# Geunwoo-Jeon/LarvaNet

Hardware: AMD Instinct MI355X
Metric: HR Mpixels/s (LarvaNet x4 multi-exit train step, 48x48 LR patches) (higher is better)
Workload: dtype f32; 1 GPU; LarvaNet x4 train_step_larva M4 B4,4,4,4 48ch, batch 16 of 3x48x48 -> 3x192x192 fp32 per GPU (BASELINE config 2); global_batch=16, parallelism=dp1, hip_graph=True

## Files before the change

larvanet_amd/csrc/conv3x3_mfma.hip:

```cpp
#include "larva_common.h"
#include "larva_bicubic.h"
#include <hip/hip_ext.h>
#include <cstdlib>
#include <type_traits>

#ifndef LARVA_DIAG
#define LARVA_DIAG 0
#endif
constexpr int kWgPerCu = 2;
constexpr int kOperandDepth = 2;


#ifndef LARVA_DIAG_ONLY48
#define LARVA_DIAG_ONLY48 0
#endif

namespace larva {

#if defined(LARVA_DIAG) && (LARVA_DIAG & 32)
__device__ unsigned long long* g_stamps = nullptr;
#if LARVA_DIAG & 512
constexpr int kDiagWgPerSlot = 256;
__device__ int g_slot_of_launch = 0;
__device__ __forceinline__ void stamp_slot(unsigned long long* area, int k) {
// ... 236 lines not shown

template <int COUT, typename G>
__device__ __forceinline__ void reg_load(const ConvArgs& a, const ChunkSrc& cs, int y0, int x0, int tid,
                                         RegStaging<COUT, G>& st) {
  using C = ConvCfg<COUT, G>;
  const size_t plane = (size_t)a.H * a.pitch;
#pragma unroll
  for (int i = 0; i < C::RIN_ITERS; ++i) {
    const int s = min(tid + i * 256, C::RIN_SLOTS - 1);
    const int ci = s / (G::HALO * (G::RS / 4));
    const int rem = s - ci * (G::HALO * (G::RS / 4));
    const int r = rem / (G::RS / 4);
    const int q = rem - r * (G::RS / 4);
    const int gy = y0 - 1 + r, gx = x0 - 4 + 4 * q;
    const bool row_ok = gy >= 0 && gy < a.H;
    const float* row = cs.img_ptr + (size_t)ci * plane + (size_t)min(max(gy, 0), a.H - 1) * a.pitch;
    f32x4 v;
#pragma unroll
    for (int e = 0; e < 4; ++e) {
      const int x = gx + e;
      const float t = row[min(max(x, 0), a.W - 1)];
      v[e] = (row_ok && x >= 0 && x < a.W) ? t : 0.f;
    }
    st.in[i] = v;
  }
#pragma unroll
  for (int i = 0; i < C::RW_ITERS; ++i) {
    const int s = min(tid + i * 256, C::RW_SLOTS - 1);
    const float* p = cs.wgt_ptr + 4 * s;
    st.w[i] = f32x4{p[0], p[1], p[2], p[3]};
  }
}

template <int COUT, typename G>
__device__ __forceinline__ void reg_store(float* stage, int tid, const RegStaging<COUT, G>& st) {
  using C = ConvCfg<COUT, G>;
#pragma unroll
  for (int i = 0; i < C::RIN_ITERS; ++i) {
    const int s = tid + i * 256;
    if (s < C::RIN_SLOTS) {
      const int ci = s / (G::HALO * (G::RS / 4));
      const int rem = s - ci * (G::HALO * (G::RS / 4));
      const int r = rem / (G::RS / 4);
      const int q = rem - r * (G::RS / 4);
      *reinterpret_cast<f32x4*>(stage + ci * C::PS + r * G::RS + 4 * q) = st.in[i];
    }
  }
#pragma unroll
  for (int i = 0; i < C::RW_ITERS; ++i) {
    const int s = tid + i * 256;
    if (s < C::RW_SLOTS) *reinterpret_cast<f32x4*>(stage + C::IN_FLOATS + 4 * s) = st.w[i];
  }
}

template <int COUT, typename G, int NCT, int PG0, int NPG>
__device__ __forceinline__ void read_operands(const float* const (&a_base)[NCT], const float* b_base, int step,
                                              float (&av)[NCT], float (&bv)[NPG]) {
  using C = ConvCfg<COUT, G>;
  if constexpr ((LARVA_DIAG & 128) != 0) {
#pragma unroll
    for (int c = 0; c < NCT; ++c) av[c] = (float)step;
#pragma unroll
    for (int p = 0; p < NPG; ++p) bv[p] = (float)(step + p);
    return;
  }
  const int tap = step / (kCh / 4), kk = step % (kCh / 4);
  const int ky = tap / 3, kx = tap % 3;
#pragma unroll
  for (int c = 0; c < NCT; ++c) av[c] = a_base[c][(tap * kCh + kk * 4) * C::CS];
#pragma unroll
  for (int p = 0; p < NPG; ++p) {
    const int pg = PG0 + p, prow = pg / G::PC, pcol = pg % G::PC;
    bv[p] = b_base[kk * 4 * C::PS + (prow + ky) * G::RS + pcol * 16 + kx];
  }
}

template <int NMF, int NRD, int M>
__device__ __forceinline__ void shadow_groups() {
  if constexpr (M < NMF) {
    __builtin_amdgcn_sched_group_barrier(0x8, 1, 0);
    constexpr int share = (NRD + NMF - 1 - M) / NMF;
    if constexpr (share > 0) __builtin_amdgcn_sched_group_barrier(0x100, share, 0);
    shadow_groups<NMF, NRD, M + 1>();
  }
}

template <int COUT, typename G, int NCT, int PG0, int NPG, bool SWAP>
__device__ __forceinline__ void mfma_chunk(const float* stage, int ct0, int lane, f32x4 (&acc)[NCT][NPG],
                                           const float* wstage = nullptr) {
  using C = ConvCfg<COUT, G>;
  const int lr = lane & 15, lq = lane >> 4;
  const float* const wrows = wstage ? wstage : stage + C::IN_FLOATS;
  const float* a_base[NCT];
#pragma unroll
  for (int c = 0; c < NCT; ++c)
    a_base[c] = wrows + lq * C::CS + lr + (cout_swizzled(COUT) ? (((ct0 + c) ^ (lq & 1)) * 16) : (ct0 + c) * 16);
  const float* b_base = stage + lq * C::PS + lr + 3;
  constexpr int D = kOperandDepth;
  float av[D + 1][NCT], bv[D + 1][NPG];
#pragma unroll
  for (int d = 0; d < D; ++d)
    if (d < C::STEPS) read_operands<COUT, G, NCT, PG0, NPG>(a_base, b_base, d, av[d], bv[d]);
#pragma unroll
  for (int step = 0; step < C::STEPS; ++step) {
    __builtin_amdgcn_sched_barrier(0);
    if (step + D < C::STEPS)
      read_operands<COUT, G, NCT, PG0, NPG>(a_base, b_base, step + D, av[(step + D) % (D + 1)], bv[(step + D) % (D + 1)]);
    constexpr int NMF = NCT * NPG;
    constexpr int NRD = NCT + NPG;
#pragma unroll
    for (int m = 0; m < NMF; ++m) {
      const float wv = av[step % (D + 1)][m / NPG], xv = bv[step % (D + 1)][m % NPG];
      acc[m / NPG][m % NPG] = __builtin_amdgcn_mfma_f32_16x16x4f32(SWAP ? xv : wv, SWAP ? wv : xv, acc[m / NPG][m % NPG], 0, 0, 0);
    }
    shadow_groups<NMF, NRD, 0>();
    __builtin_amdgcn_sched_barrier(0);
  }
}

template <int KEEP, int PIECES, int AUX>
__device__ __forceinline__ void wait_and_barrier() {
  static_assert(KEEP == PIECES + AUX, "a ring wait keeps exactly the next chunk's pieces and the operand loads in flight");
  asm volatile("; LARVA_RING pieces=%1 aux=%2\n\ts_waitcnt vmcnt(%0)\n\ts_barrier" ::"n"(KEEP), "n"(PIECES), "n"(AUX) : "memory");
  __builtin_amdgcn_sched_barrier(0);
}

template <typename G>
__device__ __forceinline__ void decode_tile(const ConvArgs& a, int vb, int& n, int& y0, int& x0) {
  const int tile = xcd_remap(vb, a.nwg);
  const int t2 = div_by_magic(tile, a.magic_tx);
  const int tx = tile - t2 * a.tiles_x;
  n = div_by_magic(t2, a.magic_ty);
  const int ty = t2 - n * a.tiles_y;
  x0 = tx * G::COLS;
  y0 = ty * G::ROWS;
}

template <int COUT, typename G, bool VEC, int EPI, int NCT, int PG0, int NPG, bool PERSIST>
struct RoleTraits {
  using C = ConvCfg<COUT, G>;
  static_assert(!VEC || C::LOADER, "the 16-byte path runs with a loader wave (2 * PIECES <= 63 for every instantiated shape)");
  static_assert(!PERSIST || VEC, "persistent tiles: the loader-wave path");
  static constexpr bool kShuffleEpi = (EPI == kEpiShuffle || EPI == kEpiShuffleBase || EPI == kEpiShuffleL1);
  static constexpr bool kPixMajor = VEC && !kShuffleEpi;
  static constexpr int NAUX = (EPI == kEpiMask || EPI == kEpiRes1 || EPI == kEpiShuffleBase)
                                  ? 1 : ((EPI == kEpiRes2 || EPI == kEpiShuffleL1) ? 2 : 0);
  static constexpr int NU = NCT * NPG;
  static constexpr int kEarlyPairs = PERSIST && COUT == 48 ? (NAUX * NU < 7 ? NAUX * NU : 7) : NAUX * NU;
  static constexpr int kLatePart = 4, kEarlyAll = 5;
  static constexpr bool kAuxLate = VEC && !kShuffleEpi && !(LARVA_DIAG & 6) && NAUX > 0 && !PERSIST;
  static constexpr int kAuxLoads = kAuxLate ? NAUX * NCT * NPG : 0;
};

template <int EPI, typename Aux>
__device__ __forceinline__ float fuse_element(float o, const Aux& aux, int c, int p, int r) {
  if constexpr (EPI == kEpiRelu) o = o < 0.f ? 0.f : o;
  if constexpr (EPI == kEpiMask) o = (aux[0][c][p][r] <= 0.f) ? 0.f : o;
  if constexpr (EPI == kEpiRes1 || EPI == kEpiRes2) o += aux[0][c][p][r];
  if constexpr (EPI == kEpiRes2) o += aux[1][c][p][r];
  return o;
}

template <int COUT, typename G, bool VEC, int EPI, int NCT, int PG0, int NPG, bool PERSIST = false>
__device__ __forceinline__ void run_role(const ConvArgs& a, float* smem, int ct0, int wave, int n, int y0, int x0, int tid) {
  using C = ConvCfg<COUT, G>;
  using T = RoleTraits<COUT, G, VEC, EPI, NCT, PG0, NPG, PERSIST>;
  constexpr bool kShuffleEpi = T::kShuffleEpi, kPixMajor = T::kPixMajor;
  constexpr int NAUX = T::NAUX;
  const int lane = tid & 63;
  const int lr = lane & 15, lq = lane >> 4;
  float* const out_ptr = a.out;
  struct { int H, W, pitch, plain; } k = {a.H, a.W, a.pitch, a.plain_stores};
  asm volatile("" : "+s"(k.H), "+s"(k.W), "+s"(k.pitch), "+s"(k.plain));

  f32x4 bias[NCT];
#pragma unroll
  for (int c = 0; c < NCT; ++c) bias[c] = f32x4{0.f, 0.f, 0.f, 0.f};
  auto load_bias = [&]() {
    if (a.bias) {
#pragma unroll
      for (int c = 0; c < NCT; ++c)
#pragma unroll
        for (int r = 0; r < 4; ++r) bias[c][r] = a.bias[(ct0 + c) * 16 + (kPixMajor ? lr : lq * 4 + r)];
    }
  };

  f32x4 aux[NAUX > 0 ? NAUX : 1][NAUX > 0 ? NCT : 1][NAUX > 0 ? NPG : 1];
  auto load_aux = [&](int part = -1) {
#pragma unroll
    for (int c = 0; c < NCT; ++c)
#pragma unroll
      for (int p = 0; p < NPG; ++p) {
        const int pg = PG0 + p, prow = pg / G::PC, pcol = pg % G::PC;
        const int y = min(y0 + prow, a.H - 1), x = min(x0 + pcol * 16 + lr, a.W - 1);
        auto want = [&](int op) {
          const int q = op * T::NU + c * NPG + p;
          return part < 0 ? true : part == T::kLatePart ? q >= T::kEarlyPairs : q < T::kEarlyPairs;
        };
        if constexpr (kShuffleEpi) {
          const int HH = 4 * a.H, WW = 4 * a.W;
          const size_t idx = (((size_t)n * C::CT + (ct0 + c)) * HH + (4 * y + lq)) * WW + 4 * x;
          if (want(0)) aux[0][c][p] = *reinterpret_cast<const f32x4*>(a.base + idx);
          if constexpr (EPI == kEpiShuffleL1) {
            if (want(1)) aux[1][c][p] = *reinterpret_cast<const f32x4*>(a.truth + idx);
          }
        } else if constexpr (kPixMajor && (PERSIST || G::COLS == 16)) {
          const unsigned plane = (unsigned)a.H * (unsigned)a.pitch;
          const unsigned lane_off = 4u * ((unsigned)lr * plane + (unsigned)lq * 4u);
          const int soff = __builtin_amdgcn_readfirstlane(
              (int)(4u * ((unsigned)((ct0 + c) * 16) * plane + (unsigned)(y0 + prow) * (unsigned)a.pitch + (unsigned)(x0 + pcol * 16))));
          auto image = [&](const float* t) {
            const unsigned long long b = reinterpret_cast<unsigned long long>(t + (size_t)n * COUT * plane);
            const unsigned lo = (unsigned)__builtin_amdgcn_readfirstlane((int)(unsigned)b);
            const unsigned hi = (unsigned)__builtin_amdgcn_readfirstlane((int)(unsigned)(b >> 32));
            return __builtin_amdgcn_make_buffer_rsrc(reinterpret_cast<void*>(((unsigned long long)hi << 32) | lo), 0,
                                                     (int)(COUT * plane * 4u), 0x00020000);
          };
          if constexpr (EPI == kEpiMask) {
            if (want(0)) aux[0][c][p] = __builtin_bit_cast(f32x4, __builtin_amdgcn_raw_buffer_load_b128(image(a.mask), lane_off, soff, 0));
          }
          if constexpr (EPI == kEpiRes1 || EPI == kEpiRes2) {
            if (want(0)) aux[0][c][p] = __builtin_bit_cast(f32x4, __builtin_amdgcn_raw_buffer_load_b128(image(a.res0), lane_off, soff, 0));
          }
          if constexpr (EPI == kEpiRes2) {
            if (want(1)) aux[1][c][p] = __builtin_bit_cast(f32x4, __builtin_amdgcn_raw_buffer_load_b128(image(a.res1), lane_off, soff, 0));
          }
        } else if constexpr (kPixMajor) {
          const size_t plane = (size_t)a.H * a.pitch;
          const int xb = min(x0 + pcol * 16 + lq * 4, a.pitch - 4);
          const size_t idx = ((size_t)n * COUT + (ct0 + c) * 16 + lr) * plane + (size_t)y * a.pitch + xb;
          if constexpr (EPI == kEpiMask) {
            if (want(0)) aux[0][c][p] = *reinterpret_cast<const f32x4*>(a.mask + idx);
          }
          if constexpr (EPI == kEpiRes1 || EPI == kEpiRes2) {
            if (want(0)) aux[0][c][p] = *reinterpret_cast<const f32x4*>(a.res0 + idx);
          }
          if constexpr (EPI == kEpiRes2) {
            if (want(1)) aux[1][c][p] = *reinterpret_cast<const f32x4*>(a.res1 + idx);
          }
        } else {
          const size_t plane = (size_t)a.H * a.pitch;
          const size_t idx0 = ((size_t)n * COUT + (ct0 + c) * 16 + lq * 4) * plane + (size_t)y * a.pitch + x;
#pragma unroll
          for (int r = 0; r < 4; ++r) {
            if constexpr (EPI == kEpiMask) aux[0][c][p][r] = a.mask[idx0 + r * plane];
            if constexpr (EPI == kEpiRes1 || EPI == kEpiRes2) aux[0][c][p][r] = a.res0[idx0 + r * plane];
            if constexpr (EPI == kEpiRes2) aux[1][c][p][r] = a.res1[idx0 + r * plane];
          }
        }
      }
  };
  auto load_early = [&]() {
    load_bias();
    if constexpr (NAUX > 0 && !T::kAuxLate && !(LARVA_DIAG & 4)) load_aux();
  };
  int pstage = 0;
  for (int vb = blockIdx.x;; vb += gridDim.x) {
  if constexpr (PERSIST) {
    if (vb >= a.nwg) break;
    decode_tile<G>(a, vb, n, y0, x0);
  }
  if constexpr (!VEC || (LARVA_DIAG & 2)) load_early();

  f32x4 acc[NCT][NPG];
#pragma unroll
  for (int c = 0; c < NCT; ++c)
#pragma unroll
    for (int p = 0; p < NPG; ++p) acc[c][p] = f32x4{0.f, 0.f, 0.f, 0.f};

  if constexpr (PERSIST) {
    load_bias();
    const int my_chunk = a.n_chunks >= 4 ? (wave & 3) : 0;
    __builtin_amdgcn_sched_barrier(0);
    for (int chunk = 0; chunk < a.n_chunks; ++chunk) {
      asm volatile("s_barrier" ::: "memory");
      __builtin_amdgcn_sched_barrier(0);
      if constexpr (NAUX > 0) {
        if (chunk == my_chunk) load_aux(T::kEarlyAll);
        __builtin_amdgcn_sched_barrier(0);
      }
      mfma_chunk<COUT, G, NCT, PG0, NPG, kPixMajor>(smem + pstage * C::STAGE_FLOATS, ct0, lane, acc);
      pstage = pstage == C::NST - 1 ? 0 : pstage + 1;
    }
    asm volatile("s_waitcnt vmcnt(0)" ::: "memory");
    __builtin_amdgcn_sched_barrier(0);
    if constexpr (T::kEarlyPairs < NAUX * T::NU) {
      load_aux(T::kLatePart);
      __builtin_amdgcn_sched_barrier(0);
    }
  } else if constexpr (VEC) {
    DmaPlan<COUT, G> pl;
    const int last = a.n_chunks - 1;
    if constexpr (!(LARVA_DIAG & 2)) {
      const ChunkSrc cs0 = chunk_src<COUT, G>(a, 0, n);
      const unsigned st0 = lds_addr_of(smem), st1 = lds_addr_of(smem + C::STAGE_FLOATS);
      stamp(6);
      make_plan<COUT, G, true>(a, wave, lane, y0, x0, pl);
#pragma unroll
      for (int i = 0; i < C::NPW; ++i)
        if (wave + 4 * i >= C::IN_PIECES) dma_piece<COUT, G>(pl, i, wave, cs0, st0);
      __builtin_amdgcn_sched_barrier(0);
      stamp(7);
      load_early();
      stamp(14);
      make_plan<COUT, G, false>(a, wave, lane, y0, x0, pl);
#pragma unroll
      for (int i = 0; i < C::NPW; ++i)
        if (wave + 4 * i < C::IN_PIECES) dma_piece<COUT, G>(pl, i, wave, cs0, st0);
      stamp(15);
      const ChunkSrc cs1 = chunk_src<COUT, G>(a, min(1, last), n);
#pragma unroll
      for (int i = 0; i < C::NPW; ++i) dma_piece<COUT, G>(pl, i, wave, cs1, st1);
      if constexpr (T::kAuxLate) {
        __builtin_amdgcn_sched_barrier(0);
        load_aux();
        __builtin_amdgcn_sched_barrier(0);
      }
    }
    stamp(1);
    int stage = 0;
    for (int chunk = 0; chunk <= last; ++chunk) {
      if constexpr ((LARVA_DIAG & 256) != 0) {
      } else if (chunk == 0) wait_and_barrier<((LARVA_DIAG & 2) ? 0 : C::NPW) + T::kAuxLoads, ((LARVA_DIAG & 2) ? 0 : C::NPW), T::kAuxLoads>();
      else wait_and_barrier<T::kAuxLoads, 0, T::kAuxLoads>();
      if (chunk == 0) stamp(2);
      stamp(8 + (chunk < 7 ? chunk : 7));
      if constexpr (!(LARVA_DIAG & 1)) mfma_chunk<COUT, G, NCT, PG0, NPG, kPixMajor>(smem + stage * C::STAGE_FLOATS, ct0, lane, acc);
      stage = stage == C::NST - 1 ? 0 : stage + 1;
    }
    asm volatile("s_waitcnt vmcnt(0)" ::: "memory");
    stamp(3);
  } else {
    RegStaging<COUT, G> st;
    if constexpr (!(LARVA_DIAG & 2)) {
      reg_load<COUT, G>(a, chunk_src<COUT, G>(a, 0, n), y0, x0, tid, st);
      reg_store<COUT, G>(smem, tid, st);
    }
    __syncthreads();
    for (int chunk = 0; chunk < a.n_chunks; ++chunk) {
      float* cur = smem + (chunk & 1) * C::STAGE_FLOATS;
      float* nxt = smem + ((chunk & 1) ^ 1) * C::STAGE_FLOATS;
      const bool more = chunk + 1 < a.n_chunks;
      if constexpr (!(LARVA_DIAG & 2)) {
        if (more) reg_load<COUT, G>(a, chunk_src<COUT, G>(a, chunk + 1, n), y0, x0, tid, st);
      }
      if constexpr (!(LARVA_DIAG & 1)) mfma_chunk<COUT, G, NCT, PG0, NPG, kPixMajor>(cur, ct0, lane, acc);
      if constexpr (!(LARVA_DIAG & 2)) {
        if (more) reg_store<COUT, G>(nxt, tid, st);
      }
      __syncthreads();
    }
  }

  if constexpr ((LARVA_DIAG & 4) != 0) {
#pragma unroll
    for (int c = 0; c < NCT; ++c)
#pragma unroll
      for (int p = 0; p < NPG; ++p) asm volatile("" ::"v"(acc[c][p]));
    return;
  }

  if constexpr (EPI == kEpiShuffleL1) {
    const int HH = 4 * k.H, WW = 4 * k.W;
    const size_t plane = (size_t)k.H * k.pitch;
    const float g = a.gval;
    float s = 0.f;
#pragma unroll
    for (int c = 0; c < NCT; ++c)
#pragma unroll
      for (int p = 0; p < NPG; ++p) {
        const int pg = PG0 + p, prow = pg / G::PC, pcol = pg % G::PC;
        const int y = y0 + prow, x = x0 + pcol * 16 + lr;
        const f32x4 v = (acc[c][p] + bias[c]) + aux[0][c][p];
        if (y < k.H && x < k.W) {
          if (out_ptr) {
            const size_t idx = (((size_t)n * C::CT + (ct0 + c)) * HH + (4 * y + lq)) * WW + 4 * x;
            __builtin_nontemporal_store(v, reinterpret_cast<f32x4*>(out_ptr + idx));
          }
          const f32x4 d = v - aux[1][c][p];
          s += fabsf(d[0]) + fabsf(d[1]) + fabsf(d[2]) + fabsf(d[3]);
          const size_t idx0 = ((size_t)n * COUT + (ct0 + c) * 16 + lq * 4) * plane + (size_t)y * k.pitch + x;
#pragma unroll
          for (int r = 0; r < 4; ++r)
            __builtin_nontemporal_store(d[r] > 0.f ? g : (d[r] < 0.f ? -g : 0.f), &a.grad[idx0 + r * plane]);
        }
      }
#pragma unroll
    for (int o = 32; o > 0; o >>= 1) s += __shfl_xor(s, o);
    if (lane == 0) a.partial[4 * blockIdx.x + wave] = s;
  } else if constexpr (EPI == kEpiShuffle || EPI == kEpiShuffleBase) {
    const int HH = 4 * k.H, WW = 4 * k.W;
#pragma unroll
    for (int c = 0; c < NCT; ++c)
#pragma unroll
      for (int p = 0; p < NPG; ++p) {
        const int pg = PG0 + p, prow = pg / G::PC, pcol = pg % G::PC;
        const int y = y0 + prow, x = x0 + pcol * 16 + lr;
        const size_t idx = (((size_t)n * C::CT + (ct0 + c)) * HH + (4 * y + lq)) * WW + 4 * x;
        f32x4 v = acc[c][p] + bias[c];
        if constexpr (EPI == kEpiShuffleBase) v += aux[0][c][p];
        if (y < k.H && x < k.W) __builtin_nontemporal_store(v, reinterpret_cast<f32x4*>(out_ptr + idx));
      }
  } else if constexpr (kPixMajor) {
    const size_t plane = (size_t)k.H * k.pitch;
    auto store_all = [&](auto plain_tag, auto interior_tag) {
      constexpr bool kPlain = decltype(plain_tag)::value;
      constexpr bool kInterior = decltype(interior_tag)::value;
#pragma unroll
      for (int c = 0; c < NCT; ++c)
#pragma unroll
        for (int p = 0; p < NPG; ++p) {
          const int pg = PG0 + p, prow = pg / G::PC, pcol = pg % G::PC;
          const int y = y0 + prow, xb = x0 + pcol * 16 + lq * 4;
          const size_t idx = ((size_t)n * COUT + (ct0 + c) * 16 + lr) * plane + (size_t)y * k.pitch + xb;
          f32x4 v = acc[c][p] + bias[c];
          if (kInterior || (y < k.H && xb < k.pitch)) {
#pragma unroll
            for (int r = 0; r < 4; ++r) {
              const float o = fuse_element<EPI>(v[r], aux, c, p, r);
              v[r] = (kInterior || xb + r < k.W) ? o : 0.f;
            }
            if constexpr (kPlain) *reinterpret_cast<f32x4*>(out_ptr + idx) = v;
            else __builtin_nontemporal_store(v, reinterpret_cast<f32x4*>(out_ptr + idx));
          }
        }
    };
    constexpr bool kFastPath = EPI == kEpiPlain || EPI == kEpiRelu || EPI == kEpiRes1;
    const bool interior = kFastPath && y0 + G::ROWS <= k.H && x0 + G::COLS <= k.W;
    auto store_policy = [&](auto plain_tag) {
      if constexpr (kFastPath) {
        if (interior) {
          store_all(plain_tag, std::true_type{});
          return;
        }
      }
      store_all(plain_tag, std::false_type{});
    };
    if constexpr ((LARVA_DIAG & 16) != 0) {
      store_policy(std::true_type{});
    } else if constexpr (G::COLS == 16) {
      if (k.plain) store_policy(std::true_type{});
      else store_policy(std::false_type{});
    } else {
      store_policy(std::false_type{});
    }
  } else {
    const size_t plane = (size_t)k.H * k.pitch;
#pragma unroll
    for (int c = 0; c < NCT; ++c)
#pragma unroll
      for (int p = 0; p < NPG; ++p) {
        const int pg = PG0 + p, prow = pg / G::PC, pcol = pg % G::PC;
        const int y = y0 + prow, x = x0 + pcol * 16 + lr;
        const size_t idx0 = ((size_t)n * COUT + (ct0 + c) * 16 + lq * 4) * plane + (size_t)y * k.pitch + x;
        const f32x4 v = acc[c][p] + bias[c];
        if (y < k.H && x < k.pitch) {
          const bool real = x < k.W;
#pragma unroll
          for (int r = 0; r < 4; ++r) {
            float o = fuse_element<EPI>(v[r], aux, c, p, r);
            o = real ? o : 0.f;
            if constexpr ((LARVA_DIAG & 16) != 0) out_ptr[idx0 + r * plane] = o;
            else __builtin_nontemporal_store(o, &out_ptr[idx0 + r * plane]);
          }
        }
      }
  }
#if LARVA_DIAG & 32
  stamp(4);
  asm volatile("s_waitcnt vmcnt(0)" ::: "memory");
  stamp(5);
#endif
  if constexpr (!PERSIST) break;
  }
}

__device__ __forceinline__ void fetch_args(const ConvArgs& a) {
  asm volatile("" ::"s"(a.src[0]), "s"(a.wpk), "s"(a.bias), "s"(a.out), "s"(a.cin_per_src), "s"(a.n_chunks), "s"(a.N),
               "s"(a.H), "s"(a.W), "s"(a.pitch), "s"(a.tiles_x), "s"(a.tiles_y), "s"(a.magic_tx), "s"(a.magic_ty),
               "s"(a.magic_cps), "s"(a.nwg), "s"(a.tile_tab), "s"(a.plain_stores), "s"(a.tab_n),
               "s"(a.tab16[0]), "s"(a.tab16[16]));
}

template <int COUT, bool VEC, int EPI, typename G = GeoWide, bool GIVEN = false>
__device__ __forceinline__ void conv_tile(const ConvArgs& a, float* smem, int wave = 0, int n = 0, int y0 = 0, int x0 = 0, int tid = 0) {
  static_assert(COUT == 48 || COUT == 32 || COUT == 64, "unsupported channel count");
  if constexpr (!GIVEN) {
    if constexpr ((LARVA_DIAG & 8) != 0) return;
    stamp(0);
    fetch_args(a);
    const int tile = xcd_remap(blockIdx.x, a.nwg);
    const int t2 = div_by_magic(tile, a.magic_tx);
    const int tx = tile - t2 * a.tiles_x;
    n = div_by_magic(t2, a.magic_ty);
    const int ty = t2 - n * a.tiles_y;
    x0 = tx * G::COLS, y0 = ty * G::ROWS;
    tid = threadIdx.x;
    wave = __builtin_amdgcn_readfirstlane(tid >> 6);
    __builtin_amdgcn_s_setprio(1);
  }
  if constexpr (VEC) {
    if (wave == 4) {
      if constexpr (GIVEN || !(LARVA_DIAG & 2)) run_loader<COUT, G>(a, smem, tid & 63, n, y0, x0);
      return;
    }
  }
  if constexpr (G::COLS == 16) {
    static_assert(VEC && ConvCfg<COUT, G>::LOADER, "the strip kernel is launched with a loader wave");
    if constexpr (COUT == 64) {
      run_role<COUT, G, VEC, EPI, 1, 0, G::ROWS>(a, smem, wave, wave, n, y0, x0, tid);
    } else if constexpr (COUT == 48) {
      if (wave < 3) run_role<COUT, G, VEC, EPI, 1, 0, G::ROWS - 1>(a, smem, wave, wave, n, y0, x0, tid);
      else run_role<COUT, G, VEC, EPI, 3, G::ROWS - 1, 1>(a, smem, 0, wave, n, y0, x0, tid);
    } else if constexpr (G::ROWS == 5) {
      if (wave < 2) run_role<COUT, G, VEC, EPI, 1, 0, 3>(a, smem, wave, wave, n, y0, x0, tid);
      else if (wave == 2) run_role<COUT, G, VEC, EPI, 2, 3, 1>(a, smem, 0, wave, n, y0, x0, tid);
      else run_role<COUT, G, VEC, EPI, 2, 4, 1>(a, smem, 0, wave, n, y0, x0, tid);
    } else {
      if (wave < 2) run_role<COUT, G, VEC, EPI, 1, 0, 2>(a, smem, wave, wave, n, y0, x0, tid);
      else run_role<COUT, G, VEC, EPI, 1, 2, 2>(a, smem, wave - 2, wave, n, y0, x0, tid);
    }
  } else if constexpr (G::ROWS == 4) {
    static_assert(VEC && (COUT == 48 || COUT == 32), "4 x 48 tiles: the 16-byte path at 48 / 32 channels");
    if constexpr (COUT == 48) {
      if (wave < 3) run_role<COUT, G, VEC, EPI, 1, 0, 9>(a, smem, wave, wave, n, y0, x0, tid);
      else run_role<COUT, G, VEC, EPI, 3, 9, 3>(a, smem, 0, wave, n, y0, x0, tid);
    } else {
      if (wave < 2) run_role<COUT, G, VEC, EPI, 1, 0, 6>(a, smem, wave, wave, n, y0, x0, tid);
      else run_role<COUT, G, VEC, EPI, 1, 6, 6>(a, smem, wave - 2, wave, n, y0, x0, tid);
    }
  } else if constexpr (COUT == 48) {
    if (wave < 3) run_role<COUT, G, VEC, EPI, 1, 0, 7>(a, smem, wave, wave, n, y0, x0, tid);
    else run_role<COUT, G, VEC, EPI, 3, 7, 2>(a, smem, 0, wave, n, y0, x0, tid);
  } else if constexpr (COUT == 32) {
    if (wave < 2) run_role<COUT, G, VEC, EPI, 1, 0, 5>(a, smem, wave, wave, n, y0, x0, tid);
    else run_role<COUT, G, VEC, EPI, 1, 5, 4>(a, smem, wave - 2, wave, n, y0, x0, tid);
  } else {
    run_role<COUT, G, VEC, EPI, 1, 0, 9>(a, smem, wave, wave, n, y0, x0, tid);
  }
}

template <int COUT, bool VEC, int EPI>
__global__ __launch_bounds__(VEC ? ConvCfg<COUT>::THREADS_DMA : 256, VEC ? kWgPerCu : 1) void conv3x3_mfma_kernel(ConvArgs a) {
  extern __shared__ __attribute__((aligned(16))) float smem[];
  conv_tile<COUT, VEC, EPI>(a, smem);
}

template <int COUT, int EPI>
__global__ __launch_bounds__((ConvCfg<COUT, GeoWide4>::THREADS_DMA), kWgPerCu) void conv3x3_mfma_rows4_kernel(ConvArgs a) {
  extern __shared__ __attribute__((aligned(16))) float smem[];
  conv_tile<COUT, true, EPI, GeoWide4>(a, smem);
}
static_assert(2 * ConvCfg<48, GeoWide4>::LDS_BYTES_DMA <= 160 * 1024, "two 4 x 48 workgroups per CU");

template <int COUT, typename G>
__device__ __forceinline__ void run_loader_persist(const ConvArgs& a, float* smem, int lane) {
  using C = ConvCfg<COUT, G>;
  static_assert(C::NST == 3 && 2 * C::PIECES <= 63, "three stages, two chunks in flight");
  LoaderPlan<COUT, G> pl;
  int vb_i = blockIdx.x, n_i, y0, x0, c_i = 0, s_i = 0;
  decode_tile<G>(a, vb_i, n_i, y0, x0);
  make_loader_plan<COUT, G>(a, lane, y0, x0, pl);
  bool more = true;
  auto issue = [&]() {
    const ChunkSrc cs = chunk_src<COUT, G>(a, c_i, n_i);
    const unsigned dst = lds_addr_of(smem + s_i * C::STAGE_FLOATS);
#pragma unroll
    for (int p = 0; p < C::PIECES; ++p)
      lds_dma16_buf(p < C::IN_PIECES ? cs.img : cs.wgt, pl.voff[p], 0, dst + 1024u * (unsigned)p);
    s_i = s_i == C::NST - 1 ? 0 : s_i + 1;
    if (++c_i == a.n_chunks) {
      c_i = 0;
      vb_i += gridDim.x;
      more = vb_i < a.nwg;
      if (more) {
        decode_tile<G>(a, vb_i, n_i, y0, x0);
        make_loader_plan<COUT, G>(a, lane, y0, x0, pl);
      }
    }
  };
  int ahead = 0;
  issue();
  ++ahead;
  if (more) {
    issue();
    ++ahead;
  }
  while (ahead > 0) {
    if (ahead == 2) asm volatile("s_waitcnt vmcnt(%0)" ::"n"(C::PIECES) : "memory");
    else asm volatile("s_waitcnt vmcnt(0)" ::: "memory");
    asm volatile("s_barrier" ::: "memory");
    __builtin_amdgcn_sched_barrier(0);
    --ahead;
    if (more) {
      issue();
      ++ahead;
    }
  }
}

template <int COUT, int EPI>
__global__ __launch_bounds__((ConvCfg<COUT>::THREADS_DMA), kWgPerCu) void conv3x3_mfma_persist_kernel(ConvArgs a) {
  extern __shared__ __attribute__((aligned(16))) float smem[];
  using G = GeoWide;
  stamp(0);
  fetch_args(a);
  const int tid = threadIdx.x;
  const int wave = __builtin_amdgcn_readfirstlane(tid >> 6);
  __builtin_amdgcn_s_setprio(1);
  if (wave == 4) {
    run_loader_persist<COUT, G>(a, smem, tid & 63);
    return;
  }
  if constexpr (COUT == 48) {
    if (wave < 3) run_role<COUT, G, true, EPI, 1, 0, 7, true>(a, smem, wave, wave, 0, 0, 0, tid);
    else run_role<COUT, G, true, EPI, 3, 7, 2, true>(a, smem, 0, wave, 0, 0, 0, tid);
  } else if constexpr (COUT == 32) {
    if (wave < 2) run_role<COUT, G, true, EPI, 1, 0, 5, true>(a, smem, wave, wave, 0, 0, 0, tid);
    else run_role<COUT, G, true, EPI, 1, 5, 4, true>(a, smem, wave - 2, wave, 0, 0, 0, tid);
  } else {
    static_assert(COUT == 64, "unsupported channel count");
    run_role<COUT, G, true, EPI, 1, 0, 9, true>(a, smem, wave, wave, 0, 0, 0, tid);
  }
}

template <int COUT, int EPI>
__global__ __launch_bounds__(320, kWgPerCu) void conv3x3_mfma_strip_kernel(ConvArgs a) {
  extern __shared__ __attribute__((aligned(16))) float smem[];
  stamp(0);
  fetch_args(a);
  const int tile = xcd_remap(blockIdx.x, a.nwg);
  const int n = div_by_magic(tile, a.magic_tx);
  const int slot = tile - n * a.tiles_x;
  unsigned e;
  if (a.tab_n) {
    const unsigned pair = (unsigned)a.tab16[slot >> 1];
    const unsigned h = (slot & 1) ? pair >> 16 : pair & 0xffffu;
    e = (h & 0xffu) | (((h >> 8) & 0x7fu) << 16) | ((h >> 15) << 31);
  } else {
    e = a.tile_tab[slot];
  }
  const int y0 = (int)(e & 0xfffu), x0 = (int)((e >> 12) & 0xfffu);
  const int tid = threadIdx.x;
  const int wave = __builtin_amdgcn_readfirstlane(tid >> 6);
  __builtin_amdgcn_s_setprio(1);
  if (e >> 31) conv_tile<COUT, true, EPI, GeoS5, true>(a, smem, wave, n, y0, x0, tid);
  else conv_tile<COUT, true, EPI, GeoS4, true>(a, smem, wave, n, y0, x0, tid);
}
template <int COUT>
constexpr size_t kStripLdsBytes = ConvCfg<COUT, GeoS5>::LDS_BYTES_DMA > ConvCfg<COUT, GeoS4>::LDS_BYTES_DMA ? ConvCfg<COUT, GeoS5>::LDS_BYTES_DMA
                                                                                                            : ConvCfg<COUT, GeoS4>::LDS_BYTES_DMA;
static_assert(kWgPerCu * kStripLdsBytes<48> <= 160 * 1024 && kWgPerCu * kStripLdsBytes<64> <= 160 * 1024, "strip workgroups per CU");

constexpr int kMaxConvJobs = 4;
struct ConvBatch {
  ConvArgs job[kMaxConvJobs];
};

template <int COUT, int EPI>
__global__ __launch_bounds__(ConvCfg<COUT>::THREADS_DMA, kWgPerCu) void conv3x3_mfma_batch_kernel(ConvBatch b) {
  extern __shared__ __attribute__((aligned(16))) float smem[];
  conv_tile<COUT, true, EPI>(b.job[blockIdx.y], smem);
}

constexpr int kMaxPackJobs = 64;

struct PackJob {
  const float* w;
  float* fwd;
  float* bwd;
  int cout, cin, w_cin_total, w_cin_off;
};

struct PackBatch {
  PackJob job[kMaxPackJobs];
};

__host__ __device__ constexpr int packed_floats(int cout, int cin) {
  return (cin / kCh) * 9 * kCh * cout_stride(cout);
}

constexpr int kPackTileCols = 64;
constexpr int kPackLd = kPackTileCols + 1;
constexpr int kPackTileFloats = 9 * kCh * kPackLd;

__host__ __device__ constexpr int pack_slots(int cout, int cin) { return cin / kCh + cout / kCh; }

__device__ __forceinline__ void pack_block(const PackJob& j, int slot, float* __restrict__ tile) {
  const int nfc = j.cin / kCh;
  const bool fwd = slot < nfc;
  const int chunk = fwd ? slot : slot - nfc;
  float* __restrict__ out = fwd ? j.fwd : j.bwd;
  if ((!fwd && chunk >= j.cout / kCh) || !out) return;
  const int cols = fwd ? j.cout : j.cin;
  const int cs = cout_stride(cols);
  const int tid = threadIdx.x;
  out += (size_t)chunk * 72 * cs;
  for (int c0 = 0; c0 < cs; c0 += kPackTileCols) {
    const int ncol = min(kPackTileCols, cols - c0);
    if (fwd) {
      for (int idx = tid; idx < ncol * 72; idx += 256) {
        const int c = idx / 72, r = idx - c * 72, k = r / 9, tap = r - k * 9;
        const int cin_abs = j.w_cin_off + chunk * kCh + k;
        tile[(tap * kCh + k) * kPackLd + c] =
            cin_abs < j.w_cin_total ? j.w[((size_t)(c0 + c) * j.w_cin_total + cin_abs) * 9 + tap] : 0.f;
      }
    } else {
      const int row = ncol * 9;
      for (int idx = tid; idx < kCh * row; idx += 256) {
        const int k = idx / row, rem = idx - k * row, c = rem / 9, tap = rem - c * 9;
        tile[((8 - tap) * kCh + k) * kPackLd + c] =
            j.w_cin_off + c0 + c < j.w_cin_total
                ? j.w[((size_t)(chunk * kCh + k) * j.w_cin_total + j.w_cin_off + c0) * 9 + rem] : 0.f;
      }
    }
    __syncthreads();
    const int wcols = min(kPackTileCols, cs - c0);
    const bool swz = cout_swizzled(cols);
    for (int idx = tid; idx < 72 * wcols; idx += 256) {
      const int r = idx / wcols, c = idx - r * wcols;
      const int col = swz ? ((c0 + c) ^ ((r & 1) << 4)) : c0 + c;
      out[r * cs + col] = c < ncol ? tile[r * kPackLd + c] : 0.f;
    }
    __syncthreads();
  }
}

__global__ __launch_bounds__(256) void pack_weights_batch_kernel(PackBatch b) {
  __shared__ float tile[kPackTileFloats];
  pack_block(b.job[blockIdx.y], blockIdx.x, tile);
}

constexpr int kPrologueBlocks = 192;
constexpr int kProloguePadSlices = 2, kPrologueBicSlices = 8;
struct PrologueArgs {
  PackBatch packs;
  int npack, slots;
  const float* x;
  float* x16;
  float* base;
  int N, C, H, W;
};

__global__ __launch_bounds__(256) void step_prologue_kernel(PrologueArgs a) {
  __shared__ float tile[kPackTileFloats];
  int blk = blockIdx.x;
  if (blk < a.npack * a.slots) {
    const int job = blk / a.slots;
    pack_block(a.packs.job[job], blk - job * a.slots, tile);
    return;
  }
  blk -= a.npack * a.slots;
  constexpr int nthr = kPrologueBlocks * 256;
  const int slice = blk / kPrologueBlocks, tid = (blk - slice * kPrologueBlocks) * 256 + threadIdx.x;
  const int nbic = a.base ? kPrologueBicSlices : 0;
  if (slice < nbic) {
    bicubic4_body(a.x, a.base, a.N * a.C, a.H, a.W, (long long)slice * nthr + tid, (long long)nthr * kPrologueBicSlices);
  } else {
    const int plane = a.H * a.W, per_img = a.C * plane, total = a.N * per_img;
    for (int i = (slice - nbic) * nthr + tid; i < total; i += nthr * kProloguePadSlices) {
      const int n = i / per_img, r = i - n * per_img;
      a.x16[(size_t)n * 16 * plane + r] = a.x[i];
    }
  }
}

struct LaunchTiming {
  hipEvent_t start, stop;
};

template <auto Kernel, typename Args>
static hipError_t launch(dim3 grid, dim3 block, size_t lds, hipStream_t stream, const LaunchTiming* tm, const Args& a) {
  static PerDeviceOnce lds_set;
  if (const hipError_t e = ensure_dynamic_lds(lds_set, reinterpret_cast<const void*>(Kernel), lds); e != hipSuccess) return e;
  if (tm)
    hipExtLaunchKernelGGL(Kernel, grid, block, lds, stream, tm->start, tm->stop, 0, a);
  else
    hipLaunchKernelGGL(Kernel, grid, block, lds, stream, a);
  return hipGetLastError();
}

template <int... E>
struct EpiSet {
  static constexpr bool has(int epi) { return ((epi == E) || ...); }
};
using EpiAll = EpiSet<kEpiPlain, kEpiRelu, kEpiMask, kEpiRes1, kEpiRes2, kEpiShuffle, kEpiShuffleBase>;
using EpiBatch48 = EpiSet<kEpiPlain, kEpiRelu, kEpiMask, kEpiRes1, kEpiRes2, kEpiShuffle, kEpiShuffleBase, kEpiShuffleL1>;
using EpiInference = EpiSet<kEpiPlain, kEpiRelu, kEpiRes1, kEpiRes2, kEpiShuffle, kEpiShuffleBase>;
using EpiRows4 = EpiInference;
using EpiPersist = EpiInference;

template <int... E, typename F>
static hipError_t with_epi(EpiSet<E...>, int epi, hipError_t absent, F&& f) {
  hipError_t r = absent;
  (void)((epi == E && (r = f(std::integral_constant<int, E>{}), true)) || ...);
  return r;
}

template <typename F>
static hipError_t with_cout(int cout, hipError_t absent, F&& f) {
  switch (cout) {
#if !LARVA_DIAG_ONLY48
    case 32: return f(std::integral_constant<int, 32>{});
    case 64: return f(std::integral_constant<int, 64>{});
#endif
    case 48: return f(std::integral_constant<int, 48>{});
    default: return absent;
  }
}

static int conv_slots() { return kWgPerCu * device_cu_count(); }

template <int COUT>
static hipError_t launch_conv(const ConvArgs& a, bool vec, int epi, hipStream_t stream, const LaunchTiming* tm) {
  using C = ConvCfg<COUT>;
  const dim3 grid(a.N * a.tiles_x * a.tiles_y);
  return with_epi(EpiAll{}, epi, hipErrorInvalidValue, [&](auto e) {
    constexpr int EPI = decltype(e)::value;
    if (vec)
      return launch<conv3x3_mfma_kernel<COUT, true, EPI>>(grid, dim3(C::THREADS_DMA), C::LDS_BYTES_DMA, stream, tm, a);
    return launch<conv3x3_mfma_kernel<COUT, false, EPI>>(grid, dim3(256), C::LDS_BYTES_REG, stream, tm, a);
  });
}

template <int COUT>
static hipError_t launch_rows4(const ConvArgs& a, int epi, hipStream_t stream, const LaunchTiming* tm) {
  using C = ConvCfg<COUT, GeoWide4>;
  return with_epi(EpiRows4{}, epi, hipErrorNotSupported, [&](auto e) {
    return launch<conv3x3_mfma_rows4_kernel<COUT, decltype(e)::value>>(dim3(a.nwg), dim3(C::THREADS_DMA), C::LDS_BYTES_DMA,
                                                                      stream, tm, a);
  });
}

template <int COUT>
static hipError_t launch_persist(const ConvArgs& a, int epi, hipStream_t stream, const LaunchTiming* tm) {
  using C = ConvCfg<COUT>;
  if ((long long)COUT * a.H * a.pitch * 4 >= (1ll << 31)) return hipErrorNotSupported;
  const int grid = a.nwg < conv_slots() ? a.nwg : conv_slots();
  return with_epi(EpiPersist{}, epi, hipErrorNotSupported, [&](auto e) {
    return launch<conv3x3_mfma_persist_kernel<COUT, decltype(e)::value>>(dim3(grid), dim3(C::THREADS_DMA), C::LDS_BYTES_DMA,
                                                                        stream, tm, a);
  });
}

template <int COUT>
static hipError_t launch_batch(const ConvBatch& b, int njobs, int epi, hipStream_t stream) {
  using C = ConvCfg<COUT>;
  using Set = std::conditional_t<COUT == 48, EpiBatch48, EpiAll>;
  const ConvArgs& a = b.job[0];
  return with_epi(Set{}, epi, epi == kEpiShuffleL1 ? hipErrorNotSupported : hipErrorInvalidValue, [&](auto e) {
    return launch<conv3x3_mfma_batch_kernel<COUT, decltype(e)::value>>(dim3(a.N * a.tiles_x * a.tiles_y, njobs),
                                                                      dim3(C::THREADS_DMA), C::LDS_BYTES_DMA, stream,
                                                                      nullptr, b);
  });
}

template <int COUT>
static hipError_t launch_strip(const ConvArgs& a, int epi, hipStream_t stream, const LaunchTiming* tm) {
  return with_epi(EpiAll{}, epi, hipErrorInvalidValue, [&](auto e) {
    return launch<conv3x3_mfma_strip_kernel<COUT, decltype(e)::value>>(dim3(a.nwg), dim3(320), kStripLdsBytes<COUT>, stream,
                                                                      tm, a);
  });
}

}

using namespace larva;

extern "C" {

long long larva_packed_weight_floats(int cout, int cin) { return (long long)packed_floats(cout, cin); }

static int fill_pack_jobs(PackBatch& b, const float* const* w, float* const* wpk_fwd, float* const* wpk_bwd,
                          const int* cout, const int* cin, const int* w_cin_total, const int* w_cin_off, int njobs) {
  int slots = 0;
  for (int i = 0; i < njobs; ++i) {
    if (!w[i] || cout[i] % kCh || cin[i] % kCh || cout[i] <= 0 || cin[i] <= 0) return -1;
    b.job[i] = PackJob{w[i], wpk_fwd[i], wpk_bwd[i], cout[i], cin[i], w_cin_total[i], w_cin_off[i]};
    const int n = pack_slots(cout[i], cin[i]);
    slots = n > slots ? n : slots;
  }
  return slots;
}

int larva_pack_weights_batch(const float* const* w, float* const* wpk_fwd, float* const* wpk_bwd,
                             const int* cout, const int* cin, const int* w_cin_total,
                             const int* w_cin_off, int njobs, void* stream) {
  if (njobs < 1 || njobs > kMaxPackJobs) return (int)hipErrorInvalidValue;
  PackBatch b{};
  const int slots = fill_pack_jobs(b, w, wpk_fwd, wpk_bwd, cout, cin, w_cin_total, w_cin_off, njobs);
  if (slots < 1) return (int)hipErrorInvalidValue;
  hipLaunchKernelGGL(pack_weights_batch_kernel, dim3(slots, njobs), dim3(256), 0, (hipStream_t)stream, b);
  return (int)hipGetLastError();
}

int larva_step_prologue(const float* const* w, float* const* wpk_fwd, float* const* wpk_bwd, const int* cout,
                        const int* cin, const int* w_cin_total, const int* w_cin_off, int njobs, const float* x,
                        float* x16, float* base, int N, int C, int H, int W, void* stream) {
  if (njobs < 0 || njobs > kMaxPackJobs || !x || N <= 0 || C <= 0 || C > 16 || H <= 0 || W <= 0)
    return (int)hipErrorInvalidValue;
  if ((long long)N * 16 * H * W >= (1ll << 31)) return (int)hipErrorInvalidValue;
  if (base && (reinterpret_cast<uintptr_t>(base) & 15)) return (int)hipErrorInvalidValue;
  PrologueArgs a{};
  a.slots = njobs ? fill_pack_jobs(a.packs, w, wpk_fwd, wpk_bwd, cout, cin, w_cin_total, w_cin_off, njobs) : 0;
  if (a.slots < 0) return (int)hipErrorInvalidValue;
  a.npack = njobs;
  a.x = x; a.x16 = x16; a.base = base;
  a.N = N; a.C = C; a.H = H; a.W = W;
  if (!x16 && base) return (int)hipErrorInvalidValue;
  const int blocks = njobs * a.slots + kPrologueBlocks * ((base ? kPrologueBicSlices : 0) + (x16 ? kProloguePadSlices : 0));
  if (blocks == 0) return 0;
  hipLaunchKernelGGL(step_prologue_kernel, dim3(blocks), dim3(256), 0, (hipStream_t)stream, a);
  return (int)hipGetLastError();
}

int larva_pack_weights(const float* w, float* wpk_fwd, float* wpk_bwd, int cout, int cin,
                       int w_cin_total, int w_cin_off, void* stream) {
  return larva_pack_weights_batch(&w, &wpk_fwd, &wpk_bwd, &cout, &cin, &w_cin_total, &w_cin_off, 1, stream);
}

#if LARVA_DIAG & 512
static int g_diag_next_slot = -1, g_diag_slot_cap = 0;
static unsigned long long* g_diag_host_base = nullptr;
static int diag_take_slot() {
  if (g_diag_next_slot < 0 || g_diag_next_slot >= g_diag_slot_cap) return -1;
  return g_diag_next_slot++;
}
int larva_diag_arm_slots(int first, int cap) {
  const int was = g_diag_next_slot;
  g_diag_next_slot = first;
  g_diag_slot_cap = cap;
  return was;
}
int larva_diag_next_slot(void) { return g_diag_next_slot; }
#endif

static int conv_build(const float* const* src, int n_src, int cin_per_src, const float* wpk, const float* bias,
                      const float* res0, const float* res1, const float* mask, const float* base, float* out,
                      int N, int H, int W, int pitch, int relu, int mode, ConvArgs& a, bool& aligned, int& epi) {
  if (pitch == 0) pitch = W;
  if (pitch < W) return (int)hipErrorInvalidValue;
  if (n_src < 1 || n_src > kMaxSrc || cin_per_src % kCh || cin_per_src <= 0 || N <= 0 || H <= 0 || W <= 0)
    return (int)hipErrorInvalidValue;
  if (mode != 0 && mode != 1) return (int)hipErrorInvalidValue;
  if ((long long)cin_per_src * H * pitch >= (1ll << 31)) return (int)hipErrorInvalidValue;
  if (!wpk || !out) return (int)hipErrorInvalidValue;
  a = ConvArgs{};
#if LARVA_DIAG & 512
  {
    const int slot = diag_take_slot();
    a.diag_area = (slot >= 0 && g_diag_host_base) ? g_diag_host_base + (size_t)slot * kDiagWgPerSlot * 16 : nullptr;
  }
#endif
  aligned = (pitch % 4 == 0) && ((reinterpret_cast<uintptr_t>(wpk) & 15) == 0);
  for (int i = 0; i < n_src; ++i) {
    if (!src[i]) return (int)hipErrorInvalidValue;
    a.src[i] = src[i];
    aligned = aligned && ((reinterpret_cast<uintptr_t>(src[i]) & 15) == 0);
  }
  aligned = aligned && (((reinterpret_cast<uintptr_t>(out) | reinterpret_cast<uintptr_t>(res0) |
                          reinterpret_cast<uintptr_t>(res1) | reinterpret_cast<uintptr_t>(mask)) & 15) == 0);
  a.wpk = wpk; a.bias = bias; a.res0 = res0; a.res1 = res1; a.mask = mask; a.base = base;
  a.out = out;
  a.cin_per_src = cin_per_src;
  a.n_chunks = n_src * cin_per_src / kCh;
  a.N = N; a.H = H; a.W = W; a.pitch = pitch;
  a.tiles_x = (pitch + kTileCols - 1) / kTileCols;
  a.tiles_y = (H + kTileRows - 1) / kTileRows;
  if ((long long)N * a.tiles_x * a.tiles_y >= (1ll << 20)) return (int)hipErrorInvalidValue;
  a.magic_tx = div_magic(a.tiles_x);
  a.magic_ty = div_magic(a.tiles_y);
  a.magic_cps = div_magic(cin_per_src / kCh);
  a.nwg = N * a.tiles_x * a.tiles_y;
  if (mode == 1) {
    if (relu || mask || res0 || res1) return (int)hipErrorInvalidValue;
    if ((reinterpret_cast<uintptr_t>(out) | reinterpret_cast<uintptr_t>(base)) & 15) return (int)hipErrorInvalidValue;
    epi = base ? kEpiShuffleBase : kEpiShuffle;
  } else {
    if (base) return (int)hipErrorInvalidValue;
    const int code = (relu ? 1 : 0) | (mask ? 2 : 0) | (res0 ? 4 : 0) | (res1 ? 8 : 0);
    switch (code) {
      case 0: epi = kEpiPlain; break;
      case 1: epi = kEpiRelu; break;
      case 2: epi = kEpiMask; break;
      case 4: epi = kEpiRes1; break;
      case 12: epi = kEpiRes2; break;
      default: return (int)hipErrorInvalidValue;
    }
  }
  return 0;
}

static int conv_tile_rows(int N, int H, int pitch, int cout, int epi, bool aligned, int forced) {
  const bool can4 = aligned && (cout == 48 || cout == 32) && EpiRows4::has(epi);
  if (forced == 3 || !can4) return 3;
  if (forced == 4) return 4;
  const long long tiles3 = (long long)N * ((pitch + kTileCols - 1) / kTileCols) * ((H + 2) / 3);
  return (cout == 32 && tiles3 > conv_slots()) ? 4 : 3;
}

static int conv_dispatch(const float* const* src, int n_src, int cin_per_src, const float* wpk,
                         const float* bias, const float* res0, const float* res1, const float* mask,
// ... 210 lines not shown
```

Baseline: 361.9 HR Mpixels/s.

## Walk batched 48-channel conv jobs with persistent workgroups and a shared loader

Adds a persistent batch kernel for 48-channel multi-exit convolutions. A fixed grid of workgroups walks the tiles of every job in sequence, with a loader wave that carries its DMA pipeline across job boundaries. The goal is to cut tail effects and per-workgroup startup compared with the one-workgroup-per-tile 2D grid. The cost is more complex index bookkeeping, including the partial-sum index now keyed by tile, and it only applies to the relu, mask and shuffle-L1 epilogues when there are more tiles than slots.

```diff
diff --git a/larvanet_amd/csrc/conv3x3_mfma.hip b/larvanet_amd/csrc/conv3x3_mfma.hip
--- a/larvanet_amd/csrc/conv3x3_mfma.hip
+++ b/larvanet_amd/csrc/conv3x3_mfma.hip
@@ -412,6 +412,10 @@
   static constexpr int kAuxLoads = kAuxLate ? NAUX * NCT * NPG : 0;
 };
 
+struct TileWalk {
+  int vb, stage;
+};
+
 template <int EPI, typename Aux>
 __device__ __forceinline__ float fuse_element(float o, const Aux& aux, int c, int p, int r) {
   if constexpr (EPI == kEpiRelu) o = o < 0.f ? 0.f : o;
@@ -421,8 +425,10 @@
   return o;
 }
 
-template <int COUT, typename G, bool VEC, int EPI, int NCT, int PG0, int NPG, bool PERSIST = false>
-__device__ __forceinline__ void run_role(const ConvArgs& a, float* smem, int ct0, int wave, int n, int y0, int x0, int tid) {
+template <int COUT, typename G, bool VEC, int EPI, int NCT, int PG0, int NPG, bool PERSIST = false, bool BATCH = false>
+__device__ __forceinline__ void run_role(const ConvArgs& a, float* smem, int ct0, int wave, int n, int y0, int x0, int tid,
+                                         TileWalk* walk = nullptr) {
+  static_assert(!BATCH || PERSIST, "the jobs of a batched launch are walked by persistent workgroups");
   using C = ConvCfg<COUT, G>;
   using T = RoleTraits<COUT, G, VEC, EPI, NCT, PG0, NPG, PERSIST>;
   constexpr bool kShuffleEpi = T::kShuffleEpi, kPixMajor = T::kPixMajor;
@@ -514,10 +520,13 @@
     load_bias();
     if constexpr (NAUX > 0 && !T::kAuxLate && !(LARVA_DIAG & 4)) load_aux();
   };
-  int pstage = 0;
-  for (int vb = blockIdx.x;; vb += gridDim.x) {
+  int pstage = BATCH ? walk->stage : 0;
+  for (int vb = BATCH ? walk->vb : blockIdx.x;; vb += gridDim.x) {
   if constexpr (PERSIST) {
-    if (vb >= a.nwg) break;
+    if (vb >= a.nwg) {
+      if constexpr (BATCH) *walk = TileWalk{vb, pstage};
+      break;
+    }
     decode_tile<G>(a, vb, n, y0, x0);
   }
   if constexpr (!VEC || (LARVA_DIAG & 2)) load_early();
@@ -647,7 +656,7 @@
       }
 #pragma unroll
     for (int o = 32; o > 0; o >>= 1) s += __shfl_xor(s, o);
-    if (lane == 0) a.partial[4 * blockIdx.x + wave] = s;
+    if (lane == 0) a.partial[4 * (PERSIST ? (unsigned)vb : blockIdx.x) + wave] = s;
   } else if constexpr (EPI == kEpiShuffle || EPI == kEpiShuffleBase) {
     const int HH = 4 * k.H, WW = 4 * k.W;
 #pragma unroll
@@ -813,17 +822,29 @@
 }
 static_assert(2 * ConvCfg<48, GeoWide4>::LDS_BYTES_DMA <= 160 * 1024, "two 4 x 48 workgroups per CU");
 
-template <int COUT, typename G>
-__device__ __forceinline__ void run_loader_persist(const ConvArgs& a, float* smem, int lane) {
+template <int COUT, typename G, int NJOBS = 0>
+__device__ __forceinline__ void run_loader_persist(const ConvArgs& a, float* smem, int lane, int njobs = 1) {
   using C = ConvCfg<COUT, G>;
   static_assert(C::NST == 3 && 2 * C::PIECES <= 63, "three stages, two chunks in flight");
   LoaderPlan<COUT, G> pl;
-  int vb_i = blockIdx.x, n_i, y0, x0, c_i = 0, s_i = 0;
+  int vb_i = blockIdx.x, n_i, y0, x0, c_i = 0, s_i = 0, job_i = 0;
+  bool more = true;
+  auto next_job = [&]() {
+    if constexpr (NJOBS > 0) {
+#pragma unroll
+      for (int k = 1; k < NJOBS; ++k)
+        if (vb_i >= a.nwg && job_i + 1 < njobs) {
+          vb_i -= a.nwg;
+          ++job_i;
+        }
+    }
+    more = vb_i < a.nwg;
+  };
+  if constexpr (NJOBS > 0) next_job();
   decode_tile<G>(a, vb_i, n_i, y0, x0);
   make_loader_plan<COUT, G>(a, lane, y0, x0, pl);
-  bool more = true;
   auto issue = [&]() {
-    const ChunkSrc cs = chunk_src<COUT, G>(a, c_i, n_i);
+    const ChunkSrc cs = chunk_src<COUT, G>(NJOBS > 0 ? (&a)[__builtin_amdgcn_readfirstlane(job_i)] : a, c_i, n_i);
     const unsigned dst = lds_addr_of(smem + s_i * C::STAGE_FLOATS);
 #pragma unroll
     for (int p = 0; p < C::PIECES; ++p)
@@ -832,7 +853,7 @@
     if (++c_i == a.n_chunks) {
       c_i = 0;
       vb_i += gridDim.x;
-      more = vb_i < a.nwg;
+      next_job();
       if (more) {
         decode_tile<G>(a, vb_i, n_i, y0, x0);
         make_loader_plan<COUT, G>(a, lane, y0, x0, pl);
@@ -915,12 +936,37 @@
 constexpr int kMaxConvJobs = 4;
 struct ConvBatch {
   ConvArgs job[kMaxConvJobs];
+  int njobs;
 };
 
 template <int COUT, int EPI>
 __global__ __launch_bounds__(ConvCfg<COUT>::THREADS_DMA, kWgPerCu) void conv3x3_mfma_batch_kernel(ConvBatch b) {
   extern __shared__ __attribute__((aligned(16))) float smem[];
   conv_tile<COUT, true, EPI>(b.job[blockIdx.y], smem);
+}
+
+template <int COUT, int EPI>
+__global__ __launch_bounds__(ConvCfg<COUT>::THREADS_DMA, kWgPerCu) void conv3x3_mfma_batch_persist_kernel(ConvBatch b) {
+  extern __shared__ __attribute__((aligned(16))) float smem[];
+  static_assert(COUT == 48, "built for the 48-channel exits (27 units -> 7,7,7,6, conv_tile's 3 x 48 row)");
+  using G = GeoWide;
+  fetch_args(b.job[0]);
+  const int njobs = b.njobs;
+  const int tid = threadIdx.x;
+  const int wave = __builtin_amdgcn_readfirstlane(tid >> 6);
+  __builtin_amdgcn_s_setprio(1);
+  if (wave == 4) {
+    run_loader_persist<COUT, G, kMaxConvJobs>(b.job[0], smem, tid & 63, njobs);
+    return;
+  }
+  TileWalk walk{(int)blockIdx.x, 0};
+#pragma unroll 1
+  for (int j = 0; j < njobs; ++j) {
+    const ConvArgs& a = b.job[j];
+    if (wave < 3) run_role<COUT, G, true, EPI, 1, 0, 7, true, true>(a, smem, wave, wave, 0, 0, 0, tid, &walk);
+    else run_role<COUT, G, true, EPI, 3, 7, 2, true, true>(a, smem, 0, wave, 0, 0, 0, tid, &walk);
+    walk.vb -= a.nwg;
+  }
 }
 
 constexpr int kMaxPackJobs = 64;
@@ -1049,6 +1095,7 @@
 using EpiInference = EpiSet<kEpiPlain, kEpiRelu, kEpiRes1, kEpiRes2, kEpiShuffle, kEpiShuffleBase>;
 using EpiRows4 = EpiInference;
 using EpiPersist = EpiInference;
+using EpiBatchPersist = EpiSet<kEpiRelu, kEpiMask, kEpiShuffleL1>;
 
 template <int... E, typename F>
 static hipError_t with_epi(EpiSet<E...>, int epi, hipError_t absent, F&& f) {
@@ -1104,10 +1151,20 @@
 }
 
 template <int COUT>
-static hipError_t launch_batch(const ConvBatch& b, int njobs, int epi, hipStream_t stream) {
+static hipError_t launch_batch(ConvBatch& b, int njobs, int epi, hipStream_t stream) {
   using C = ConvCfg<COUT>;
   using Set = std::conditional_t<COUT == 48, EpiBatch48, EpiAll>;
   const ConvArgs& a = b.job[0];
+  b.njobs = njobs;
+  if constexpr (COUT == 48) {
+    const char* pe = getenv("LARVA_PERSIST");
+    if (!(pe && pe[0] == '0') && (long long)njobs * a.nwg > conv_slots() && EpiBatchPersist::has(epi) &&
+        (long long)COUT * a.H * a.pitch * 4 < (1ll << 31))
+      return with_epi(EpiBatchPersist{}, epi, hipErrorInvalidValue, [&](auto e) {
+        return launch<conv3x3_mfma_batch_persist_kernel<COUT, decltype(e)::value>>(dim3(conv_slots()), dim3(C::THREADS_DMA),
+                                                                                  C::LDS_BYTES_DMA, stream, nullptr, b);
+      });
+  }
   return with_epi(Set{}, epi, epi == kEpiShuffleL1 ? hipErrorNotSupported : hipErrorInvalidValue, [&](auto e) {
     return launch<conv3x3_mfma_batch_kernel<COUT, decltype(e)::value>>(dim3(a.N * a.tiles_x * a.tiles_y, njobs),
                                                                       dim3(C::THREADS_DMA), C::LDS_BYTES_DMA, stream,
```

Result: no change. 362.4 HR Mpixels/s (median of 3 runs) (+0.1%).
